# ielhelw/mcmc-ammsb-gpu

Hardware: AMD Instinct MI355X
Metric: mini-batch edges/s (SG-MCMC a-MMSB learner loop) (higher is better)
Workload: dtype f32

## Files before the change

### include/ammsb.h

```cpp
#ifndef AMMSB_H
#define AMMSB_H

#include <stddef.h>
#include <stdint.h>

#ifdef __cplusplus
extern "C" {
#endif

#define AMMSB_VERSION 200

enum {
  AMMSB_OK = 0,
  AMMSB_EINVAL = -1,
  AMMSB_EHIP = -2,
  AMMSB_ENOMEM = -3,
  AMMSB_ENODEV = -4,
  AMMSB_ERANGE = -5
};

#define AMMSB_MAX_GROUPS 65535u
#define AMMSB_RPM_MAX_BLOCKS 32

typedef struct { uint64_t x, y; } ammsb_seed;
// ... 38 lines not shown
int ammsb_ctx_destroy(ammsb_ctx* ctx);
int ammsb_ctx_params(const ammsb_ctx* ctx, ammsb_params* out);

int ammsb_rng_init(ammsb_ctx* ctx, ammsb_seed* seeds, uint64_t n, uint64_t sx, uint64_t sy, void* stream);
int ammsb_rng_init_mixed(ammsb_ctx* ctx, ammsb_seed* seeds, uint64_t n, uint64_t sx, uint64_t sy, void* stream);

int ammsb_set_has(ammsb_ctx* ctx, const ammsb_set* set, const uint64_t* keys, uint64_t n, uint8_t* out,
                  void* stream);

uint64_t ammsb_set_num_bins(uint64_t n);
int ammsb_set_build(ammsb_ctx* ctx, const uint64_t* keys, uint64_t n, uint64_t* slots, uint64_t num_bins,
                    uint32_t* prime_idx_out, uint32_t* scratch, void* stream);

int ammsb_pi_init_gamma(ammsb_ctx* ctx, const ammsb_rpm* pi, float* phi_sum, float eta0, float eta1,
                        ammsb_seed* seeds, void* stream);

int ammsb_sample_neighbors(ammsb_ctx* ctx, ammsb_seed* seeds, const uint32_t* nodes, uint32_t n_nodes,
                           uint32_t wg, uint32_t* table, uint32_t* packed, void* stream);

int ammsb_update_phi(ammsb_ctx* ctx, const float* beta, const ammsb_rpm* pi, const float* phi_sum,
                     const ammsb_set* training_set, const uint32_t* nodes, const uint32_t* neighbors,
                     uint32_t n_nodes, uint32_t step_count, ammsb_seed* seeds, uint32_t wg, uint32_t flags,
                     uint32_t group_begin, uint32_t group_end, float* phi_vec, void* stream);

int ammsb_update_phi_occupancy(ammsb_ctx* ctx, uint32_t wg, int* blocks_per_cu, int* waves_per_block);

int ammsb_update_pi(ammsb_ctx* ctx, const ammsb_rpm* pi, float* phi_sum, const float* phi_vec,
                    const uint32_t* nodes, uint32_t n_nodes, uint32_t wg, void* stream);

int ammsb_theta_sum(ammsb_ctx* ctx, float* out, void* stream);

int ammsb_beta_grads(ammsb_ctx* ctx, const float* theta, const float* beta, const ammsb_rpm* pi,
                     const ammsb_set* training_set, const uint64_t* edges, uint32_t n_edges,
                     uint32_t edge_begin, uint32_t edge_end, uint32_t wg, float* grads_out, void* stream);

int ammsb_can_fuse_pi_beta(ammsb_ctx* ctx, uint32_t phi_wg, uint32_t beta_wg);
int ammsb_update_pi_beta_grads(ammsb_ctx* ctx, const float* theta, const float* beta, const ammsb_rpm* pi,
                               float* phi_sum, const float* phi_vec, const uint32_t* nodes,
                               const ammsb_set* training_set, const uint64_t* edges, uint32_t n_edges, uint32_t wg,
                               float* grads_out, void* stream);

int ammsb_sum_rows_f32(ammsb_ctx* ctx, const float* in, uint32_t rows, uint32_t cols, float* out, void* stream);

int ammsb_update_theta(ammsb_ctx* ctx, float* theta, float* beta, const float* grads, uint32_t step_count,
                       float scale, ammsb_seed* seeds, uint32_t flags, void* stream);

// ... 90 lines not shown
```

### include/mcmc/operators.h

```cpp
#ifndef MCMC_AMD_OPERATORS_H_
#define MCMC_AMD_OPERATORS_H_

#include <functional>
#include <istream>
#include <memory>
#include <ostream>
#include <string>
#include <vector>

#include "ammsb.h"
#include "mcmc/config.h"
#include "mcmc/device.h"

namespace mcmc {

std::shared_ptr<ammsb_ctx> AcquireContext(const Config& cfg, const clcuda::Queue& queue);
void ThrowIfError(ammsb_ctx* ctx, int rc, const char* what);

template <class T>
class RowPartitionedMatrix {
 public:
  RowPartitionedMatrix(clcuda::Queue queue, uint32_t rows, uint32_t cols, uint32_t rows_in_block = 0);
  uint32_t Rows() const { return rows_; }
  uint32_t Cols() const { return cols_; }
// ... 137 lines not shown
    void* stop;
    uint64_t* acc;
  };
  void* Take();
  std::vector<Rec> pending_;
  std::vector<void*> free_;
  void* cur_ = nullptr;
};

class PhiUpdater {
 public:
  PhiUpdater(const Config& cfg, clcuda::Queue queue, clcuda::Buffer<Float>& beta, RowPartitionedMatrix<Float>* pi,
             clcuda::Buffer<Float>& phi, OpenClSet* trainingSet, const std::vector<std::string>& compileFlags = {},
             const std::string& baseFuncs = "");
  void operator()(clcuda::Buffer<Vertex>& mini_batch_nodes, clcuda::Buffer<Vertex>& neighbors,
                  uint32_t num_mini_batch_nodes);
  uint64_t UpdatePhiTime() const { return t_update_phi_; }
  uint64_t UpdatePiTime() const { return t_update_pi_; }
  clcuda::Buffer<Float>& GetPhiVec() { return phi_vec_; }
  void BeginCall() { ++count_calls_; }
  void UpdatePhi(clcuda::Buffer<Vertex>& nodes, clcuda::Buffer<Vertex>& neighbors, uint32_t n, uint32_t group_begin,
                 uint32_t group_end);
  void UpdatePi(clcuda::Buffer<Vertex>& nodes, uint32_t n);
  random::OpenClRandom& Rand() { return rand_; }
  uint32_t& CountCalls() { return count_calls_; }
  uint32_t Local() const { return local_; }
  uint32_t Flags() const { return flags_; }
  void ResolveTimers() { timers_.Resolve(); }
  void AddTimes(uint64_t phi_ns, uint64_t pi_ns) {
    t_update_phi_ += phi_ns;
    t_update_pi_ += pi_ns;
  }
  bool Serialize(std::ostream* out);
  bool Parse(std::istream* in);

 private:
  std::shared_ptr<ammsb_ctx> ctx_;
  clcuda::Queue queue_;
  clcuda::Buffer<Float>& beta_;
  RowPartitionedMatrix<Float>* pi_;
  clcuda::Buffer<Float>& phi_;
  OpenClSet* trainingSet_;
  uint64_t max_nodes_;
  clcuda::Buffer<Float> phi_vec_;
  random::OpenClRandom rand_;
  uint32_t count_calls_, local_, flags_;
// ... 86 lines not shown
```

### mcmc-ammsb-gpu_amd/_capi.py

```python
import ctypes as C
import os

import numpy as np

_HERE = os.path.dirname(os.path.abspath(__file__))
LIB_PATH = os.environ.get("AMMSB_HIP_LIB") or os.path.join(_HERE, "libammsb_hip.so")

RPM_MAX_BLOCKS = 32
MAX_GROUPS = 65535
NOISE_OFF = 1
PHI_STREAMING = 2


class AmmsbError(RuntimeError):
    pass


class Params(C.Structure):
    _fields_ = [("N", C.c_uint64), ("K", C.c_uint64), ("E", C.c_uint64),
                ("num_node_sample", C.c_uint32),
                ("alpha", C.c_float), ("a", C.c_float), ("b", C.c_float), ("c", C.c_float),
                ("epsilon", C.c_float), ("eta0", C.c_float), ("eta1", C.c_float)]


# ... 24 lines not shown
                ("beta_seeds", _vp), ("grads", _vp), ("beta_wg", _u32), ("beta_flags", _u32),
                ("edges", _vp * 2), ("nodes", _vp * 2), ("neighbors", _vp * 2), ("nbr_table", _vp * 2),
                ("nbr_seeds", _vp * 2), ("nbr_wg", _u32),
                ("csr_offsets", _vp), ("csr_targets", _vp), ("mb_seeds", _vp), ("mb_candidates", _u32),
                ("mb_workspace", _vp), ("mb_count", _vp), ("mini_batch", _u32), ("max_fan_out", _u32),
                ("max_nodes", _u32), ("max_edges", _u32), ("flags", _u32)]


class MbChoice(C.Structure):
    _fields_ = [("link", _u32), ("u", _u32), ("n", _u32), ("n_candidates", _u32)]


SIGNATURES = {
    "ammsb_version": [],
    "ammsb_strerror": [C.c_int],
    "ammsb_last_error": [_vp],
    "ammsb_last_kernel_name": [_vp, C.c_int],
    "ammsb_params_quantize": [_P(Params)],
    "ammsb_eps_t": [_P(Params), _u32],
    "ammsb_ctx_create": [C.c_int, _P(Params), _P(_vp)],
    "ammsb_ctx_destroy": [_vp],
    "ammsb_theta_sum": [_vp, _vp, _vp],
    "ammsb_ctx_params": [_vp, _P(Params)],
    "ammsb_rng_init": [_vp, _vp, _u64, _u64, _u64, _vp],
    "ammsb_rng_init_mixed": [_vp, _vp, _u64, _u64, _u64, _vp],
    "ammsb_set_has": [_vp, _P(SetDesc), _vp, _u64, _vp, _vp],
    "ammsb_set_num_bins": [_u64],
    "ammsb_set_build": [_vp, _vp, _u64, _vp, _u64, _P(_u32), _vp, _vp],
    "ammsb_pi_init_gamma": [_vp, _P(Rpm), _vp, _f32, _f32, _vp, _vp],
    "ammsb_sample_neighbors": [_vp, _vp, _vp, _u32, _u32, _vp, _vp, _vp],
    "ammsb_update_phi": [_vp, _vp, _P(Rpm), _vp, _P(SetDesc), _vp, _vp, _u32, _u32, _vp, _u32, _u32,
                         _u32, _u32, _vp, _vp],
    "ammsb_update_phi_occupancy": [_vp, _u32, _P(C.c_int), _P(C.c_int)],
    "ammsb_update_pi": [_vp, _P(Rpm), _vp, _vp, _vp, _u32, _u32, _vp],
    "ammsb_beta_grads": [_vp, _vp, _vp, _P(Rpm), _P(SetDesc), _vp, _u32, _u32, _u32, _u32, _vp, _vp],
    "ammsb_can_fuse_pi_beta": [_vp, _u32, _u32],
    "ammsb_update_pi_beta_grads": [_vp, _vp, _vp, _P(Rpm), _vp, _vp, _vp, _P(SetDesc), _vp, _u32, _u32, _vp, _vp],
    "ammsb_sum_rows_f32": [_vp, _vp, _u32, _u32, _vp, _vp],
    "ammsb_update_theta": [_vp, _vp, _vp, _vp, _u32, _f32, _vp, _u32, _vp],
    "ammsb_beta_from_theta": [_vp, _vp, _vp, _vp],
    "ammsb_perplexity": [_vp, _vp, _P(Rpm), _P(SetDesc), _vp, _u32, _u32, _u32, _u32, _u32, _vp, _vp, _vp],
    "ammsb_minibatch_link": [_vp, _vp, _vp, _u32, _u32, _vp, _vp, _vp],
    "ammsb_minibatch_candidates": [_u64, _u32],
    "ammsb_minibatch_candidates_for": [_u64, _u32, _u64],
    "ammsb_minibatch_workspace_bytes": [_u32],
    "ammsb_minibatch_nonlink": [_vp, _vp, _u32, _u32, _u32, _u32, _P(SetDesc), _P(SetDesc), _vp, _vp, _vp, _vp, _vp],
# ... 96 lines not shown
```

### mcmc-ammsb-gpu_amd/csrc/ammsb_core.hip

```cpp
#include <math.h>
#include <stdlib.h>
#include <string.h>

#include "ammsb_ctx.h"
#include "ammsb_dev.h"
#include "ammsb_step.h"

using namespace ammsb;


extern "C" int ammsb_version(void) { return AMMSB_VERSION; }

extern "C" const char* ammsb_strerror(int code) {
  switch (code) {
    case AMMSB_OK: return "ok";
    case AMMSB_EINVAL: return "invalid argument";
    case AMMSB_EHIP: return "HIP runtime error";
    case AMMSB_ENOMEM: return "out of device memory";
    case AMMSB_ENODEV: return "no usable gfx950 device";
    case AMMSB_ERANGE: return "size out of range for the launch shape";
    default: return "unknown error";
  }
}

// ... 58 lines not shown
  *out = ctx;
  return AMMSB_OK;
}

extern "C" int ammsb_ctx_destroy(ammsb_ctx* ctx) {
  if (!ctx) return AMMSB_EINVAL;
  (void)hipSetDevice(ctx->device);
  if (ctx->grad_partials) (void)hipFree(ctx->grad_partials);
  if (ctx->theta_sum) (void)hipFree(ctx->theta_sum);
  if (ctx->theta_coef) (void)hipFree(ctx->theta_coef);
  if (ctx->ppx_partials) (void)hipFree(ctx->ppx_partials);
  if (ctx->ppx_cnt_partials) (void)hipFree(ctx->ppx_cnt_partials);
  if (ctx->ppx_ticket) (void)hipFree(ctx->ppx_ticket);
  free(ctx);
  return AMMSB_OK;
}

extern "C" int ammsb_ctx_params(const ammsb_ctx* ctx, ammsb_params* out) {
  if (!ctx || !out) return AMMSB_EINVAL;
  *out = ctx->params;
  return AMMSB_OK;
}

static inline uint32_t div_up(uint64_t a, uint64_t b) { return (uint32_t)((a + b - 1) / b); }


__global__ void rng_init_kernel(ammsb_seed* seeds, uint64_t n, uint64_t sx, uint64_t sy) {
  for (uint64_t i = blockIdx.x * (uint64_t)blockDim.x + threadIdx.x; i < n; i += (uint64_t)gridDim.x * blockDim.x) {
    seeds[i].x = sx + i;
    seeds[i].y = sy + i;
  }
}

extern "C" int ammsb_rng_init(ammsb_ctx* ctx, ammsb_seed* seeds, uint64_t n, uint64_t sx, uint64_t sy, void* stream) {
  AMMSB_CHECK_ARG(ctx, ctx && seeds, "null argument");
  if (n == 0) return AMMSB_OK;
  const uint32_t grid = div_up(n, 256) < 4096 ? div_up(n, 256) : 4096;
  rng_init_kernel<<<grid, 256, 0, as_stream(stream)>>>(seeds, n, sx, sy);
  AMMSB_LAUNCH_CHECK(ctx);
  return AMMSB_OK;
}

__device__ __forceinline__ uint64_t splitmix64(uint64_t z) {
  z += 0x9e3779b97f4a7c15ull;
  z = (z ^ (z >> 30)) * 0xbf58476d1ce4e5b9ull;
  z = (z ^ (z >> 27)) * 0x94d049bb133111ebull;
// ... 552 lines not shown
```

### mcmc-ammsb-gpu_amd/csrc/ammsb_ctx.h

```cpp
#pragma once

#include <hip/hip_runtime.h>
#include <stdarg.h>
#include <stdint.h>
#include <stdio.h>

#include <string>

#include "../../include/ammsb.h"

struct ammsb_ctx {
  int device;
  ammsb_params params;
  int num_cus;
  float* grad_partials;
  uint32_t max_partials;
  float* theta_sum;
  float4* theta_coef;
  double* ppx_partials;
  unsigned long long* ppx_cnt_partials;
  uint32_t max_ppx_blocks;
  uint32_t* ppx_ticket;
  const char* kernel_name[7];
  char err[256];
};

enum { AMMSB_KN_PHI = 0, AMMSB_KN_PI = 1, AMMSB_KN_GRADS = 2, AMMSB_KN_PPX = 3, AMMSB_KN_PHI_SMALL = 4, AMMSB_KN_NBR = 5,
       AMMSB_KN_GRADS_SUM = 6 };

static inline std::string ammsb_kname(const char* fmt, ...) {
  char buf[128];
  va_list ap;
  va_start(ap, fmt);
  vsnprintf(buf, sizeof buf, fmt, ap);
  va_end(ap);
  return std::string(buf);
}

#define AMMSB_CHECK_ARG(ctx, cond, msg)                                   \
  do {                                                                    \
    if (!(cond)) {                                                        \
      if (ctx) snprintf((ctx)->err, sizeof((ctx)->err), "%s: %s", __func__, msg); \
      return AMMSB_EINVAL;                                                \
    }                                                                     \
  } while (0)

// ... 30 lines not shown
```

### mcmc-ammsb-gpu_amd/csrc/ammsb_dev.h

```cpp
#pragma once

#include <hip/hip_runtime.h>
#include <stdint.h>

#include "../../include/ammsb.h"

namespace ammsb {


#include "zig_tables.inc"

struct ZigTables {
#ifndef AMMSB_ZIG_YTAB_GLOBAL
  float ytab[128];
#endif
  float wtab[128];
  uint32_t ktab[128];
};

__device__ __forceinline__ void zig_load(ZigTables* t) {
  for (int i = threadIdx.x; i < 128; i += blockDim.x) {
#ifndef AMMSB_ZIG_YTAB_GLOBAL
    t->ytab[i] = zig_ytab[i];
#endif
// ... 185 lines not shown
  FastMod mod;
  uint32_t prime_idx;
};
inline __host__ DevSet dev_set(const ammsb_set& s) {
  return DevSet{s.slots, s.num_bins, fast_mod_init(s.num_bins ? s.num_bins : 1), s.prime_idx};
}

struct SetProbe {
  ulonglong2 a0, a1, c0, c1;
};
__device__ __forceinline__ SetProbe set_probe(const DevSet& set, uint64_t k) {
  const uint64_t h1 = fast_mod(kSetPrimes[2 * set.prime_idx] * k, set.mod);
  const uint64_t h2 = fast_mod(k ^ kSetPrimes[2 * set.prime_idx + 1], set.mod);
  const ulonglong2* b1 = reinterpret_cast<const ulonglong2*>(set.slots + h1 * 4);
  const ulonglong2* b2 = reinterpret_cast<const ulonglong2*>(set.slots + (set.num_bins + h2) * 4);
  return SetProbe{b1[0], b1[1], b2[0], b2[1]};
}
__device__ __forceinline__ bool set_hit(const SetProbe& p, uint64_t k) {
  return (p.a0.x == k) | (p.a0.y == k) | (p.a1.x == k) | (p.a1.y == k) | (p.c0.x == k) | (p.c0.y == k) |
         (p.c1.x == k) | (p.c1.y == k);
}
__device__ __forceinline__ bool set_has(const DevSet& set, uint64_t k) { return set_hit(set_probe(set, k), k); }


__device__ __forceinline__ float* rpm_row(const ammsb_rpm& m, uint64_t row) {
#ifdef AMMSB_RPM_SINGLE
  return reinterpret_cast<float*>(m.blocks[0]) + row * m.num_cols;
#endif
  if (m.num_blocks == 1) return reinterpret_cast<float*>(m.blocks[0]) + row * m.num_cols;
  const uint32_t r = (uint32_t)row, rib = (uint32_t)m.rows_in_block;
  const uint32_t blk = r / rib;
  const uint64_t off = (uint64_t)(r - blk * rib) * m.num_cols;
  return reinterpret_cast<float*>(m.blocks[blk]) + off;
}


template <int L>
struct Group {
  static_assert(L >= 1 && L <= 1024 && (L & (L - 1)) == 0, "L must be a power of two <= 1024");
  static constexpr int BLOCK = L < 64 ? 64 : L;
  static constexpr int PER_BLOCK = BLOCK / L;
  static constexpr int AUX = L > 64 ? 2 * L : 1;

  __device__ __forceinline__ static int lane() { return threadIdx.x & (L - 1); }
  __device__ __forceinline__ static int slot() { return threadIdx.x / L; }

// ... 227 lines not shown
```

### mcmc-ammsb-gpu_amd/csrc/ammsb_phi.hip

```cpp
#pragma clang fp contract(off)

#include <stdlib.h>

#include "ammsb_ctx.h"
#include "ammsb_dev.h"
#include "ammsb_step.h"

#include <type_traits>

using namespace ammsb;

#ifdef AMMSB_PHI_TRACE
__device__ unsigned long long g_phi_trace[256];
#define PHI_TRACE(slot) do { if (blockIdx.x == 0 && threadIdx.x == 0 && (slot) < 256) g_phi_trace[(slot)] = __builtin_readcyclecounter(); } while (0)
extern "C" int ammsb_debug_trace(unsigned long long* out, int n) {
  return hipMemcpyFromSymbol(out, HIP_SYMBOL(g_phi_trace), sizeof(unsigned long long) * (n < 256 ? n : 256)) == hipSuccess ? 0 : -2;
}
#define AMMSB_PHI_BLK_CAP 65536
__device__ unsigned long long g_phi_blk[AMMSB_PHI_BLK_CAP * 5];
#define PHI_BLK(end) do { if (threadIdx.x == 0 && blockIdx.x < AMMSB_PHI_BLK_CAP) { \
    g_phi_blk[blockIdx.x * 5 + (end)] = __builtin_readcyclecounter(); \
    g_phi_blk[blockIdx.x * 5 + 2 + (end)] = __builtin_amdgcn_s_memrealtime(); \
    if (!(end)) g_phi_blk[blockIdx.x * 5 + 4] = (unsigned long long)__builtin_amdgcn_s_getreg((31 << 11) | 4) | \
                                               ((unsigned long long)__builtin_amdgcn_s_getreg((31 << 11) | 20) << 32); } } while (0)
// ... 7 lines not shown

#ifndef AMMSB_PHI_LDS3_DEFAULT
#define AMMSB_PHI_LDS3_DEFAULT false
#endif

namespace {

struct PhiArgs {
  const float* beta;
  ammsb_rpm pi;
  const float* phi_sum;
  DevSet set;
  const uint32_t* nodes;
  const uint32_t* neighbors;
  ammsb_seed* seeds;
  float* phi_vec;
  uint32_t n_nodes, G, group_begin, group_end;
  uint32_t K, n;
  float eps_t, alpha, epsilon, Nn;
  uint32_t noise_on;
  uint32_t rows_nt;
  const ammsb_step_desc* desc;
  unsigned long long* stamps;
};


struct PhiStep {
  uint32_t n_nodes, G, group_end;
  float eps_t;
};
__device__ __forceinline__ PhiStep phi_step(const PhiArgs& a) {
  PhiStep st = {a.n_nodes, a.G, a.group_end, a.eps_t};
  if (a.desc) {
    st.n_nodes = a.desc->n_nodes;
    st.G = st.n_nodes < AMMSB_MAX_GROUPS ? st.n_nodes : AMMSB_MAX_GROUPS;
    st.group_end = st.G;
    st.eps_t = a.desc->eps_t;
  }
  return st;
}

template <int L, int KPT, int DEPTH, bool FULL, bool ONE = false>
__global__ __launch_bounds__(Group<L>::BLOCK) void update_phi_kernel(const PhiArgs a) {
  if constexpr (ONE) __builtin_assume(a.pi.num_blocks == 1);
  using Grp = Group<L>;
  extern __shared__ uint32_t s_nb_all[];
  __shared__ ZigTables zig;
// ... 361 lines not shown
  auto group_sum = [&](float v) -> float {
    if constexpr (W == 1) {
      return VLn::tree(v);
    } else {
      float* x = xsum + phase * L;
      phase ^= 1;
      x[tid] = v;
      __syncthreads();
      float part[W];
#pragma unroll
      for (int i = 0; i < W; ++i) part[i] = x[64 * i + ln];
#pragma unroll
      for (int st = W / 2; st >= 1; st >>= 1) {
#pragma unroll
        for (int i = 0; i < st; ++i) part[i] += part[i + st];
      }
      return Group<64>::wave_tree64(part[0]);
    }
  };

  for (uint64_t i = g; i < st.n_nodes; i += st.G) {
    const uint32_t node = a.nodes[i];
    group_sync();
    for (uint32_t q = tid; q < n; q += L) {
      const uint32_t nbq = a.neighbors[i * n + q];
      const bool y = set_has(a.set, make_edge(node, nbq));
      s_nb[q] = nbq | (y ? 0x80000000u : 0u);
    }
    group_sync();

    const float phi_sum = a.phi_sum[node];
    const float inv_phi_sum = 1.0f / phi_sum;
    const float* row_a = rpm_row(a.pi, node);
    f32x2 pi_a[HP], grads[HP], rden[HP];
    bool node_safe = beta_safe && in_range(phi_sum, kPhiSumLo, kPhiSumHi);
#pragma unroll
    for (int p = 0; p < HP; ++p)
      pi_a[p] = f32x2{__builtin_nontemporal_load(row_a + tid + 2 * L * p), __builtin_nontemporal_load(row_a + tid + 2 * L * p + L)};
#pragma unroll
    for (uint32_t r = 0; r < (uint32_t)(D - 1); ++r)
      if (r < n) request(r, r);
#pragma unroll
    for (int p = 0; p < HP; ++p) {
      grads[p] = f32x2{0.0f, 0.0f};
      const f32x2 den = pi_a[p] * phi_sum;
      rden[p] = f32x2{exact_rcp(den.x), exact_rcp(den.y)};
      node_safe = node_safe && in_range(den.x, kDenLo, kDenHi) && in_range(den.y, kDenLo, kDenHi);
      const f32x2 ep = den * st.eps_t;
      s_noise[ln + 128 * p] = sqrtf(ep.x);
      s_noise[ln + 128 * p + 64] = sqrtf(ep.y);
// ... 62 lines not shown
          f32x2 qv = div_exact3(pr, psum2, rps2);
          qv = div_exact3(qv, pi_a[p] * ps, rden[p]);
          grads[p] += qv - inv_phi_sum;
        }
      } else {
#pragma unroll
        for (int p = 0; p < HP; ++p) {
          const f32x2 den = pi_a[p] * phi_sum;
          float q0 = row[ln + 128 * p] / probs_sum;
          float q1 = row[ln + 128 * p + 64] / probs_sum;
          q0 = q0 / den.x;
          q1 = q1 / den.y;
          grads[p] += f32x2{q0 - inv_phi_sum, q1 - inv_phi_sum};
        }
      }
    }

    if (a.noise_on) {
#pragma unroll 1
      for (uint32_t j = D > 2 ? n : (n > 0 ? n - 1 : 0); j < (uint32_t)KV; ++j) draw_normal(j);
    }
    asm volatile("s_waitcnt lgkmcnt(0)" ::: "memory");

    float* out = a.phi_vec + i * K;
    const float half = st.eps_t / 2;
#pragma unroll
    for (int p = 0; p < HP; ++p) {
      const f32x2 bb = f32x2{s_noise[ln + 128 * p], s_noise[ln + 128 * p + 64]};
      const f32x2 phi_k = pi_a[p] * phi_sum;
      const f32x2 ng = grads[p] * a.Nn;
      f32x2 in = a.alpha - phi_k;
      in = in + ng;
      const f32x2 drift = in * half;
      const f32x2 aa = phi_k + drift;
      const f32x2 s2 = aa + bb;
      const float v0 = fabsf(s2.x), v1 = fabsf(s2.y);
      __builtin_nontemporal_store(v0 > 1e-24f ? v0 : 1e-24f, out + tid + 2 * L * p);
      __builtin_nontemporal_store(v1 > 1e-24f ? v1 : 1e-24f, out + tid + 2 * L * p + L);
    }
  }
  if (a.noise_on && tid < LV) a.seeds[(uint64_t)g * LV + tid] = rs;
  PHI_BLK(1);
}

template <int KPT, int VL = 64, bool ONE = false>
__global__ __launch_bounds__(64) __attribute__((amdgpu_waves_per_eu(3))) void update_phi_lds3_kernel(const PhiArgs a) {
  if constexpr (ONE) __builtin_assume(a.pi.num_blocks == 1);
  using VLn = VLane<VL>;
  constexpr int D = 3;
  constexpr int KV = KPT * VLn::PER;
  constexpr int L = 64, KW = 64 * KPT, K = L * KPT, PIECES = KPT / 4, HP = KPT / 2;
  extern __shared__ __align__(16) char smem[];
  __shared__ ZigTables zig;
  const int tid = threadIdx.x, ln = tid;
  const uint32_t n = a.n;
  float* ring = reinterpret_cast<float*>(smem);
  uint32_t* s_nb = reinterpret_cast<uint32_t*>(smem + D * KW * sizeof(float));

  const PhiStep st = phi_step(a);
  note_stamp(a.stamps, a.desc, AMMSB_STAMP_PHI);
  const uint32_t g = a.group_begin + blockIdx.x;
// ... 202 lines not shown

  auto request = [&](uint32_t q, uint32_t slot) {
    const uint32_t nbr = __builtin_amdgcn_readfirstlane(s_nb[q] & 0x7fffffffu);
    const float* src = rpm_row(a.pi, nbr) + 4 * tid;
    char* dst = smem + slot * (KW * sizeof(float));
    if (a.rows_nt) {
#pragma unroll
      for (int t = 0; t < PIECES; ++t)
        __builtin_amdgcn_global_load_lds((glb_void_t*)(src + 4 * L * t), (lds_void_t*)(dst + 1024 * t), 16, 0, 2);
    } else {
#pragma unroll
      for (int t = 0; t < PIECES; ++t)
        __builtin_amdgcn_global_load_lds((glb_void_t*)(src + 4 * L * t), (lds_void_t*)(dst + 1024 * t), 16, 0, 0);
    }
  };

  PHI_TRACE(0);
  for (uint32_t g = g0; g < st.group_end; g += gridDim.x) {
  if (a.noise_on) rs = a.seeds[(uint64_t)g * VL + VLn::vlane(tid)];
  for (uint64_t i = g; i < st.n_nodes; i += st.G) {
    const uint32_t node = a.nodes[i];
    __syncthreads();
    for (uint32_t q = tid; q < n; q += L) s_nb[q] = a.neighbors[i * n + q];
    __syncthreads();
    PHI_TRACE(1);

    const float phi_sum = a.phi_sum[node];
    const float inv_phi_sum = 1.0f / phi_sum;
    const float* row_a = rpm_row(a.pi, node);
    f32x2 pi_a[HP], grads[HP], rden[HP];
    bool node_safe = beta_safe && in_range(phi_sum, kPhiSumLo, kPhiSumHi);
#pragma unroll
    for (int p = 0; p < HP; ++p)
      pi_a[p] = f32x2{__builtin_nontemporal_load(row_a + tid + 2 * L * p), __builtin_nontemporal_load(row_a + tid + 2 * L * p + L)};
#pragma unroll
    for (uint32_t r = 0; r < (uint32_t)(D - U); ++r)
      if (r < n) request(r, r);
    const bool one_probe = n <= (uint32_t)L;
    const uint32_t my_nb = one_probe && (uint32_t)tid < n ? s_nb[tid] : 0u;
    SetProbe my_probe = {};
    if (one_probe && (uint32_t)tid < n) my_probe = set_probe(a.set, make_edge(node, my_nb));
    float zraw[REGN ? KV : 1];
    if constexpr (REGN) {
      if (a.noise_on) {
#pragma unroll
        for (int j = 0; j < KV; ++j) zraw[j] = rng_normal(rs, &zig);
      }
    }
    if (one_probe) {
      if ((uint32_t)tid < n && set_hit(my_probe, make_edge(node, my_nb))) s_nb[tid] = my_nb | 0x80000000u;
    } else {
      for (uint32_t q = tid; q < n; q += L) {
        const uint32_t nb = s_nb[q];
        if (set_has(a.set, make_edge(node, nb))) s_nb[q] = nb | 0x80000000u;
      }
    }
    __syncthreads();
    PHI_TRACE(2);
#pragma unroll
    for (int p = 0; p < HP; ++p) {
      grads[p] = f32x2{0.0f, 0.0f};
      const f32x2 den = pi_a[p] * phi_sum;
      rden[p] = f32x2{exact_rcp(den.x), exact_rcp(den.y)};
      node_safe = node_safe && in_range(den.x, kDenLo, kDenHi) && in_range(den.y, kDenLo, kDenHi);
      const f32x2 ep = den * st.eps_t;
      if constexpr (REGN) {
        nz[2 * p] = sqrtf(ep.x);
        nz[2 * p + 1] = sqrtf(ep.y);
      } else {
        s_noise[ln + 128 * p] = sqrtf(ep.x);
        s_noise[ln + 128 * p + 64] = sqrtf(ep.y);
      }
    }

    PHI_TRACE(3);
    for (uint32_t q = 0; q < n; q += U) {
      float* row[U];
// ... 433 lines not shown

  const PhiStep st = phi_step(a);
  note_stamp(a.stamps, a.desc, AMMSB_STAMP_PHI);
  const uint32_t g = a.group_begin + blockIdx.x;
  if (g >= st.group_end) return;
  const float EPS = a.epsilon;
  if (a.noise_on) zig_load(&zig);

  float bf[KPT];
  bool beta_safe = true;
#pragma unroll
  for (int j = 0; j < KPT; ++j) {
    const float b = a.beta[2 * (ln + 64 * j) + 1];
    bf[j] = b - EPS;
    beta_safe = beta_safe && in_range(b, EPS, kBetaHi);
  }
  ammsb_seed rs = {0, 0};
  const bool noise_wave = wv == RW;
  if (a.noise_on && noise_wave) rs = a.seeds[(uint64_t)g * VL + VLn::vlane(ln)];

  for (uint64_t i = g; i < st.n_nodes; i += st.G) {
    const uint32_t node = a.nodes[i];
    __syncthreads();
    for (uint32_t q = tid; q < n; q += T) {
      const uint32_t nbq = a.neighbors[i * n + q];
      const bool y = set_has(a.set, make_edge(node, nbq));
      s_nb[q] = nbq | (y ? 0x80000000u : 0u);
    }
    const float phi_sum = a.phi_sum[node];
    const float inv_phi_sum = 1.0f / phi_sum;
    const float* row_a = rpm_row(a.pi, node);
    float pi_a[KPT], rden[KPT];
    bool node_safe = beta_safe && in_range(phi_sum, kPhiSumLo, kPhiSumHi);
#pragma unroll
    for (int j = 0; j < KPT; ++j) pi_a[j] = row_a[ln + 64 * j];
    if (noise_wave) {
#pragma unroll
      for (int j = 0; j < KPT; ++j) s_pia[ln + 64 * j] = pi_a[j];
    } else {
#pragma unroll
      for (int j = 0; j < KPT; ++j) {
        const float den = pi_a[j] * phi_sum;
        rden[j] = exact_rcp(den);
        node_safe = node_safe && in_range(den, kDenLo, kDenHi);
      }
    }
    __syncthreads();

    if (!noise_wave) {
      float cur[KPT], nxt[KPT];
// ... 890 lines not shown
  if (generic && gen_threads(p.K, wg, 1) == 0) {
    snprintf(ctx->err, sizeof ctx->err, "ammsb_update_phi: K=%llu at wg=%u: more than 32 columns per work-item needs K <= %u",
             (unsigned long long)p.K, wg, kGenMaxK);
    return AMMSB_ERANGE;
  }
  PhiArgs a;
  a.beta = beta;
  a.pi = *pi;
  a.phi_sum = phi_sum;
  a.set = dev_set(*training_set);
  a.nodes = nodes;
  a.neighbors = neighbors;
  a.seeds = seeds;
  a.phi_vec = phi_vec;
  a.n_nodes = n_nodes;
  a.G = n_nodes < AMMSB_MAX_GROUPS ? n_nodes : AMMSB_MAX_GROUPS;
  a.group_begin = group_begin;
  a.group_end = group_end < a.G ? group_end : a.G;
  a.K = (uint32_t)p.K;
  a.n = p.num_node_sample;
  a.eps_t = desc ? 0.0f : ammsb_eps_t(&p, step_count);
  a.desc = desc;
  a.stamps = stamps;
  a.alpha = p.alpha;
  a.epsilon = p.epsilon;
  a.Nn = (1.0f * (float)p.N) / (float)p.num_node_sample;
  a.noise_on = (flags & AMMSB_NOISE_OFF) ? 0u : 1u;
  {
    static const int nt_mode = [] {
      const char* f = getenv("AMMSB_PHI_NT");
      return f ? atoi(f) : -1;
    }();
    const uint64_t pi_bytes = pi->num_rows * pi->num_cols * sizeof(float);
    a.rows_nt = nt_mode >= 0 ? (uint32_t)nt_mode : (pi_bytes > (256ull << 20) ? 1u : 0u);
  }
  if (a.group_begin >= a.group_end) return AMMSB_OK;
  const uint32_t n_groups = a.group_end - a.group_begin;
  hipStream_t s = as_stream(stream);
  static const bool lds3_env = [] {
    const char* f = getenv("AMMSB_PHI_LDS3");
    return f ? atoi(f) != 0 : AMMSB_PHI_LDS3_DEFAULT;
  }();
  const bool lds3 = g_phi_form_lds3 >= 0 ? g_phi_form_lds3 != 0 : lds3_env;
  static const bool force_reg = [] {
    const char* f = getenv("AMMSB_PHI_FORM");
    return f && f[0] == 'r';
// ... 199 lines not shown
```

### mcmc-ammsb-gpu_amd/host/learner.cc

```cpp
#include "mcmc/learner.h"
#include "mcmc/exchange.h"
#include "mcmc/serialize.h"
#include "ammsb_refsample.h"

#include <hip/hip_runtime.h>

#include <algorithm>
#include <chrono>
#include <cmath>
#include <cstring>
#include <functional>
#include <iostream>
#include <random>
#include <sstream>
#include <stdexcept>
#include <string>
#include <tuple>

using namespace std::chrono;

namespace mcmc {

namespace {
clcuda::Buffer<Edge> Upload(const clcuda::Queue& q, const std::vector<Edge>& v) {
// ... 58 lines not shown
    trainingPerplexity_.reset(new PerplexityCalculator(PerplexityCalculator::EDGE_PER_WORKGROUP, cfg_, queue_, beta_,
                                                       pi_.get(), *devTrainingPerplexityEdges_, trainingSet_.get()));
  }
  samples_[0].reset(new Sample(cfg_, queue_, cfg_.sample_seed[0]));
  samples_[1].reset(new Sample(cfg_, queue_, cfg_.sample_seed[1]));
  if (cfg_.sampling_stream != "own" && cfg_.sampling_stream != "reference")
    throw std::runtime_error("sampling_stream must be own or reference (got " + cfg_.sampling_stream + ")");
  ref_stream_ = cfg_.device_sampling && cfg_.sampling_stream == "reference";
  if (ref_stream_ && cfg_.graph_launch)
    throw std::runtime_error("graph_launch does not cover sampling_stream reference: the descriptor loop needs each "
                             "mini-batch's sizes before the device has drawn it");
  if (cfg_.device_sampling) {
    if (cfg_.strategy != Node && cfg_.strategy != NodeLink && cfg_.strategy != NodeNonLink)
      throw std::runtime_error("device sampling implements Node / NodeLink / NodeNonLink only");
    ctx_ = AcquireContext(cfg_, queue_);
    std::vector<uint64_t> off;
    std::vector<Vertex> tgt;
    cfg_.trainingGraph->ExportCSR(&off, &tgt);
    if (tgt.empty()) throw std::runtime_error("training graph has no edges");
    degree_.resize(cfg_.N);
    for (uint64_t u = 0; u < cfg_.N; ++u) degree_[u] = static_cast<uint32_t>(off[u + 1] - off[u]);
    csr_offsets_.reset(new clcuda::Buffer<uint64_t>(queue_.GetContext(), queue_, off.begin(), off.end()));
    csr_targets_.reset(new clcuda::Buffer<Vertex>(queue_.GetContext(), queue_, tgt.begin(), tgt.end()));
    excluded_.assign(cfg_.N, 1);
    uint32_t max_excluded = 1;
    for (uint64_t u = 0; u < cfg_.N; ++u) excluded_[u] += degree_[u];
    if (cfg_.heldout)
      for (Edge e : cfg_.heldout_edges)
        if (cfg_.heldout->Has(e)) {
          Vertex a, b;
          std::tie(a, b) = Vertices(e);
          ++excluded_[a];
          ++excluded_[b];
        }
    for (uint64_t u = 0; u < cfg_.N; ++u) max_excluded = std::max(max_excluded, excluded_[u]);
    candidates_ = CandidatesForExcluded(max_excluded);
    if (candidates_ == 0)
      throw std::runtime_error("device sampling needs N >= 2 * mini_batch with room for the largest degree");
    if (ref_stream_) {
      for (uint64_t u = 0; u < cfg_.N; ++u)
        for (uint64_t i = off[u]; i < off[u + 1]; ++i)
          if (tgt[i] == u) throw std::runtime_error("reference-stream sampling: the training graph holds a self-loop");
      const uint64_t items = std::max<uint64_t>(cfg_.mini_batch_size, cfg_.trainingGraph->MaxFanOut()) + 1;
      ammsb_refsample* h = nullptr;
      const int rc = ammsb_refsample_create(queue_.device(), cfg_.N, static_cast<uint32_t>(cfg_.mini_batch_size),
                                            candidates_, static_cast<uint32_t>(items), &h);
// ... 836 lines not shown
```

### mcmc-ammsb-gpu_amd/host/operators.cc

```cpp
#include "mcmc/operators.h"
#include "mcmc/exchange.h"
#include "mcmc/serialize.h"

#include <hip/hip_runtime.h>

#include <algorithm>
#include <iostream>
#include <cstring>
#include <map>
#include <mutex>
#include <stdexcept>
#include <tuple>

namespace mcmc {

void ThrowIfError(ammsb_ctx* ctx, int rc, const char* what) {
  if (rc == AMMSB_OK) return;
  throw std::runtime_error(std::string(what) + ": " + ammsb_strerror(rc) + " (" + ammsb_last_error(ctx) + ")");
}

std::shared_ptr<ammsb_ctx> AcquireContext(const Config& cfg, const clcuda::Queue& queue) {
  const ammsb_params p = MakeKernelParams(cfg);
  ammsb_ctx* ctx = nullptr;
  const int rc = ammsb_ctx_create(queue.device(), &p, &ctx);
// ... 268 lines not shown
  return cfg;
}

PhiUpdater::PhiUpdater(const Config& cfg, clcuda::Queue queue, clcuda::Buffer<Float>& beta,
                       RowPartitionedMatrix<Float>* pi, clcuda::Buffer<Float>& phi, OpenClSet* trainingSet,
                       const std::vector<std::string>&, const std::string&)
    : ctx_(AcquireContext(CheckedPhiConfig(cfg), queue)),
      queue_(queue),
      beta_(beta),
      pi_(pi),
      phi_(phi),
      trainingSet_(trainingSet),
      max_nodes_(MaxNodes(cfg)),
      phi_vec_(queue.GetContext(), PhiVecRows(cfg) * cfg.K),
      rand_(queue, max_nodes_ * cfg.phi_wg_size, cfg.phi_seed),
      count_calls_(0),
      local_(cfg.phi_wg_size),
      flags_(cfg.phi_disable_noise ? AMMSB_NOISE_OFF : 0u),
      async_(cfg.async_launch),
      timed_(cfg.async_launch && cfg.loop_timers && !cfg.graph_launch),
      t_update_phi_(0),
      t_update_pi_(0) {}

void PhiUpdater::operator()(clcuda::Buffer<Vertex>& nodes, clcuda::Buffer<Vertex>& neighbors, uint32_t n) {
  if (n == 0) throw std::runtime_error("mini-batch nodes size = 0!");
  if (n > max_nodes_) throw std::runtime_error("grads too small");
  ++count_calls_;
  if (async_) {
    if (timed_) timers_.Start(queue_.stream());
    ThrowIfError(ctx_.get(),
                 ammsb_update_phi(ctx_.get(), beta_.data(), &pi_->Get(), phi_.data(), &trainingSet_->Get(), nodes.data(),
                                  neighbors.data(), n, count_calls_, rand_.Get(), local_, flags_, 0, 0xFFFFFFFFu,
                                  phi_vec_.data(), queue_.stream()),
                 "ammsb_update_phi");
    if (timed_) {
      timers_.Stop(queue_.stream(), &t_update_phi_);
      timers_.Start(queue_.stream());
    }
    ThrowIfError(ctx_.get(),
                 ammsb_update_pi(ctx_.get(), &pi_->Get(), phi_.data(), phi_vec_.data(), nodes.data(), n, local_,
                                 queue_.stream()),
                 "ammsb_update_pi");
    if (timed_) timers_.Stop(queue_.stream(), &t_update_pi_);
    return;
  }
  {
// ... 238 lines not shown
```

### mcmc-ammsb-gpu_amd/learner.py

```python
import concurrent.futures
import os
import time

import numpy as np
import torch

from ._capi import AmmsbError, MAX_GROUPS
from .postfit import PostFit


class Config:

    def __init__(self, **kw):
        self.heldout_ratio = 0.01
        self.alpha = 0.001
        self.a, self.b, self.c = 0.0315, 1024.0, 0.5
        self.epsilon = 1e-7
        self.eta0, self.eta1 = 1.0, 1.0
        self.K = 32
        self.mini_batch_size = 32
        self.num_node_sample = 32
        self.N = 0
        self.E = 0
        self.ppx_wg_size = 32
# ... 160 lines not shown
        if cfg.sample_parallel:
            self.samples.append(Sample(self, cfg.sample_seeds[1]))
        self.phase = 0
        self.futures = [None, None]
        self.pool = (concurrent.futures.ThreadPoolExecutor(max_workers=1)
                     if not cfg.device_sampling or self.ref_stream else None)
        self.dev_sampler = None
        self.ref_sampler = None
        self.loop = None
        self._loop_dirty = False
        if cfg.device_sampling:
            off, tgt = dataset.training_csr()
            he = np.ascontiguousarray(dataset.heldout_edges, dtype=np.uint64)
            he = he[dataset.heldout.Has(he)] if he.size else he
            ends = np.concatenate([he >> np.uint64(32), he & np.uint64(0xFFFFFFFF)]).astype(np.int64)
            hdeg = np.bincount(ends, minlength=N)[:N]
            if self.ref_stream:
                self.ref_sampler = ops.ReferenceStreamSampler(c, off, tgt, self.trainingSet, self.heldoutSet,
                                                              cfg.mini_batch_size, heldout_degree=hdeg)
            else:
                self.dev_sampler = ops.DeviceMiniBatchSampler(c, off, tgt, self.trainingSet, self.heldoutSet,
                                                              cfg.mini_batch_size, cfg.device_sampling_seed,
                                                              heldout_degree=hdeg)
        self.grads_mode, self.grads_fused = "sharded", False
        if self.sharded:
            want = str(getattr(cfg, "beta_grads", "auto"))
            if want not in ("auto", "sharded", "replicated"):
                raise AmmsbError("beta_grads must be auto, sharded or replicated (got %r)" % (want,))
            fusable = (self.dev_sampler is not None and cfg.strategy in ("Node", "NodeLink", "NodeNonLink")
                       and hasattr(self.betaUpdater, "can_fuse_update_pi")
                       and self.betaUpdater.can_fuse_update_pi(self.phiUpdater))
            self.grads_mode = "replicated" if want == "replicated" or (want == "auto" and fusable) else "sharded"
            self.grads_fused = fusable
        if self.sharded:
            self.rep_stream = ops.new_stream(c)
            self.ev_fork, self.ev_join = ops.new_event(), ops.new_event()
            self.all_grads = c.zeros((self.world, 2 * K), torch.float32)
            self.grads_sum = c.zeros((2 * K,), torch.float32)
            self.all_sums = c.zeros((self.world, 4), torch.int64)
            self.tail_buf = c.zeros((max(max_nodes - MAX_GROUPS, 1), K), torch.float32)
        from . import hostlib
        self.theta.copy_(c.from_numpy(hostlib.theta_init(K, cfg.eta0, cfg.eta1)))
        ops.beta_from_theta(c, self.theta, self.beta)
        ops.RandomGammaAndNormalize(c, cfg.eta0, cfg.eta1, self.pi, self.phi)
        self.pi_placement = None
        self._place_pi()
# ... 661 lines not shown
```

### mcmc-ammsb-gpu_amd/ops.py

```python
import ctypes as C
import os
import threading

import numpy as np
import torch

from . import _capi
from ._capi import AmmsbError, NOISE_OFF, PHI_STREAMING, Params, PpxSums, Rpm, SetDesc, check

SEED_DT = np.dtype([("x", np.uint64), ("y", np.uint64)])


_tls = threading.local()


def _stream():
    stack = getattr(_tls, "stack", None)
    if stack:
        return stack[-1]
    return C.c_void_p(torch.cuda.current_stream().cuda_stream)


def _torch_stream():
    stack = getattr(_tls, "tstack", None)
# ... 58 lines not shown
        if not torch.cuda.is_available():
            raise AmmsbError("no HIP device visible: the MI355X path has no CPU fallback")
        self.lib = _capi.load()
        self.device = torch.device("cuda", torch.cuda.current_device() if device is None else device)
        self.params = params
        self._ctx = C.c_void_p()
        check(self.lib.ammsb_ctx_create(self.device.index, C.byref(params), C.byref(self._ctx)))

    @property
    def handle(self):
        return self._ctx

    def check(self, rc):
        check(rc, self._ctx)

    KERNELS = ("update_phi", "update_pi", "beta_grads", "perplexity", "update_phi_small", "sample_neighbors",
               "grads_sum")

    def kernel_names(self):
        names = {k: self.lib.ammsb_last_kernel_name(self.handle, i).decode() for i, k in enumerate(self.KERNELS)}
        if not names["update_phi"]:
            names["update_phi"] = names["update_phi_small"]
        return names

    def close(self):
        if self._ctx:
            self.lib.ammsb_ctx_destroy(self._ctx)
            self._ctx = C.c_void_p()

    def __del__(self):
        try:
            self.close()
        except Exception:
            pass

    def empty(self, shape, dtype):
        return torch.empty(shape, dtype=dtype, device=self.device)

    def zeros(self, shape, dtype):
        return torch.zeros(shape, dtype=dtype, device=self.device)

    def from_numpy(self, arr):
        a = np.ascontiguousarray(arr)
        if a.dtype == np.uint64:
            a = a.view(np.int64)
        elif a.dtype == np.uint32:
# ... 1165 lines not shown
```

Baseline: 36.33 million.

## Test phi neighbor link flags against CSR adjacency rows instead of hash set

Registers the training graph CSR (offsets/targets) with the context and, in the update_phi kernels, decides whether each sampled neighbor is a training link by scanning the node's adjacency row with wavefront readlane broadcasts and XOR-min comparisons, for rows of degree up to 256. Nodes with larger degree, and configurations with the AMMSB_PHI_FLAGS=s env override, keep the hash-set probe. The aim is to replace scattered hash-table probes with a coalesced read of one contiguous row. It adds a scan cost proportional to degree, plus kernarg reloads of the set and adjacency pointers through the kernarg segment. A small output-pointer tweak in the store loop keeps tid in a vector register.

```diff
diff --git a/include/ammsb.h b/include/ammsb.h
--- a/include/ammsb.h
+++ b/include/ammsb.h
@@ -84,6 +84,8 @@
                      const ammsb_set* training_set, const uint32_t* nodes, const uint32_t* neighbors,
                      uint32_t n_nodes, uint32_t step_count, ammsb_seed* seeds, uint32_t wg, uint32_t flags,
                      uint32_t group_begin, uint32_t group_end, float* phi_vec, void* stream);
+
+int ammsb_ctx_set_training_adjacency(ammsb_ctx* ctx, const uint64_t* offsets, const uint32_t* targets);
 
 int ammsb_update_phi_occupancy(ammsb_ctx* ctx, uint32_t wg, int* blocks_per_cu, int* waves_per_block);
 
diff --git a/include/mcmc/operators.h b/include/mcmc/operators.h
--- a/include/mcmc/operators.h
+++ b/include/mcmc/operators.h
@@ -183,6 +183,7 @@
   void UpdatePhi(clcuda::Buffer<Vertex>& nodes, clcuda::Buffer<Vertex>& neighbors, uint32_t n, uint32_t group_begin,
                  uint32_t group_end);
   void UpdatePi(clcuda::Buffer<Vertex>& nodes, uint32_t n);
+  void SetTrainingAdjacency(const uint64_t* offsets, const Vertex* targets);
   random::OpenClRandom& Rand() { return rand_; }
   uint32_t& CountCalls() { return count_calls_; }
   uint32_t Local() const { return local_; }
diff --git a/mcmc-ammsb-gpu_amd/_capi.py b/mcmc-ammsb-gpu_amd/_capi.py
--- a/mcmc-ammsb-gpu_amd/_capi.py
+++ b/mcmc-ammsb-gpu_amd/_capi.py
@@ -70,6 +70,7 @@
     "ammsb_ctx_destroy": [_vp],
     "ammsb_theta_sum": [_vp, _vp, _vp],
     "ammsb_ctx_params": [_vp, _P(Params)],
+    "ammsb_ctx_set_training_adjacency": [_vp, _vp, _vp],
     "ammsb_rng_init": [_vp, _vp, _u64, _u64, _u64, _vp],
     "ammsb_rng_init_mixed": [_vp, _vp, _u64, _u64, _u64, _vp],
     "ammsb_set_has": [_vp, _P(SetDesc), _vp, _u64, _vp, _vp],
diff --git a/mcmc-ammsb-gpu_amd/csrc/ammsb_core.hip b/mcmc-ammsb-gpu_amd/csrc/ammsb_core.hip
--- a/mcmc-ammsb-gpu_amd/csrc/ammsb_core.hip
+++ b/mcmc-ammsb-gpu_amd/csrc/ammsb_core.hip
@@ -104,6 +104,14 @@
   return AMMSB_OK;
 }
 
+extern "C" int ammsb_ctx_set_training_adjacency(ammsb_ctx* ctx, const uint64_t* offsets, const uint32_t* targets) {
+  AMMSB_CHECK_ARG(ctx, ctx, "null context");
+  AMMSB_CHECK_ARG(ctx, (offsets == nullptr) == (targets == nullptr), "offsets and targets: both or neither");
+  ctx->adj_offsets = offsets;
+  ctx->adj_targets = targets;
+  return AMMSB_OK;
+}
+
 static inline uint32_t div_up(uint64_t a, uint64_t b) { return (uint32_t)((a + b - 1) / b); }
 
 
diff --git a/mcmc-ammsb-gpu_amd/csrc/ammsb_ctx.h b/mcmc-ammsb-gpu_amd/csrc/ammsb_ctx.h
--- a/mcmc-ammsb-gpu_amd/csrc/ammsb_ctx.h
+++ b/mcmc-ammsb-gpu_amd/csrc/ammsb_ctx.h
@@ -22,6 +22,8 @@
   uint32_t max_ppx_blocks;
   uint32_t* ppx_ticket;
   const char* kernel_name[7];
+  const uint64_t* adj_offsets;
+  const uint32_t* adj_targets;
   char err[256];
 };
 
diff --git a/mcmc-ammsb-gpu_amd/csrc/ammsb_dev.h b/mcmc-ammsb-gpu_amd/csrc/ammsb_dev.h
--- a/mcmc-ammsb-gpu_amd/csrc/ammsb_dev.h
+++ b/mcmc-ammsb-gpu_amd/csrc/ammsb_dev.h
@@ -231,6 +231,46 @@
 }
 __device__ __forceinline__ bool set_has(const DevSet& set, uint64_t k) { return set_hit(set_probe(set, k), k); }
 
+constexpr uint32_t kAdjRowCap = 256;
+
+struct AdjRow {
+  const uint32_t* row;
+  uint32_t deg;
+  __device__ __forceinline__ bool usable() const { return deg <= kAdjRowCap; }
+};
+__device__ __forceinline__ AdjRow adj_row(const uint64_t* offsets, const uint32_t* targets, uint32_t node) {
+  AdjRow r = {nullptr, kAdjRowCap + 1};
+  if (offsets) {
+    typedef unsigned long long u64x2 __attribute__((ext_vector_type(2), aligned(8)));
+    const u64x2 o = *reinterpret_cast<const u64x2*>(offsets + node);
+    const uint64_t d = o.y - o.x;
+    const uint64_t p = reinterpret_cast<uint64_t>(targets + o.x);
+    const uint32_t lo = __builtin_amdgcn_readfirstlane((uint32_t)p), hi = __builtin_amdgcn_readfirstlane((uint32_t)(p >> 32));
+    r.row = reinterpret_cast<const uint32_t*>(((uint64_t)hi << 32) | lo);
+    r.deg = __builtin_amdgcn_readfirstlane(d <= kAdjRowCap ? (uint32_t)d : kAdjRowCap + 1);
+  }
+  return r;
+}
+__device__ __forceinline__ uint32_t adj_chunk(const AdjRow& r, uint32_t c0, uint32_t lane) {
+  const uint32_t k = c0 + lane;
+  return r.row[k < r.deg ? k : r.deg - 1];
+}
+__device__ __forceinline__ uint32_t adj_scan(uint32_t t, uint32_t m, uint32_t id, uint32_t miss) {
+  for (uint32_t j = 0; j < m; ++j) {
+    const uint32_t x = (uint32_t)__builtin_amdgcn_readlane((int)t, (int)j) ^ id;
+    miss = x < miss ? x : miss;
+  }
+  return miss;
+}
+__device__ __forceinline__ bool adj_has(const AdjRow& r, uint32_t lane, uint32_t id, uint32_t t0) {
+  uint32_t miss = adj_scan(t0, r.deg < 64 ? r.deg : 64, id, 0xFFFFFFFFu);
+  for (uint32_t c0 = 64; c0 < r.deg; c0 += 64) miss = adj_scan(adj_chunk(r, c0, lane), r.deg - c0 < 64 ? r.deg - c0 : 64, id, miss);
+  return miss == 0;
+}
+__device__ __forceinline__ bool adj_has(const AdjRow& r, uint32_t lane, uint32_t id) {
+  return r.deg ? adj_has(r, lane, id, adj_chunk(r, 0, lane)) : false;
+}
+
 
 __device__ __forceinline__ float* rpm_row(const ammsb_rpm& m, uint64_t row) {
 #ifdef AMMSB_RPM_SINGLE
diff --git a/mcmc-ammsb-gpu_amd/csrc/ammsb_phi.hip b/mcmc-ammsb-gpu_amd/csrc/ammsb_phi.hip
--- a/mcmc-ammsb-gpu_amd/csrc/ammsb_phi.hip
+++ b/mcmc-ammsb-gpu_amd/csrc/ammsb_phi.hip
@@ -53,7 +53,33 @@
   uint32_t rows_nt;
   const ammsb_step_desc* desc;
   unsigned long long* stamps;
+  const uint64_t* adj_offsets;
+  const uint32_t* adj_targets;
 };
+
+struct PhiFlagArgs {
+  DevSet set;
+  const uint64_t* adj_offsets;
+  const uint32_t* adj_targets;
+};
+typedef const __attribute__((address_space(4))) char* kernarg_ptr_t;
+__device__ __forceinline__ uint64_t kernarg_u64(kernarg_ptr_t ka, size_t off) {
+  return *reinterpret_cast<const __attribute__((address_space(4))) uint64_t*>(ka + off);
+}
+__device__ __forceinline__ PhiFlagArgs phi_flag_args() {
+  kernarg_ptr_t ka = (kernarg_ptr_t)__builtin_amdgcn_kernarg_segment_ptr();
+  asm volatile("" : "+s"(ka));
+  constexpr size_t S = offsetof(PhiArgs, set);
+  PhiFlagArgs f;
+  f.set.slots = reinterpret_cast<const uint64_t*>(kernarg_u64(ka, S + offsetof(DevSet, slots)));
+  f.set.num_bins = kernarg_u64(ka, S + offsetof(DevSet, num_bins));
+  f.set.mod.d = kernarg_u64(ka, S + offsetof(DevSet, mod) + offsetof(FastMod, d));
+  f.set.mod.m = kernarg_u64(ka, S + offsetof(DevSet, mod) + offsetof(FastMod, m));
+  f.set.prime_idx = (uint32_t)kernarg_u64(ka, S + offsetof(DevSet, prime_idx));
+  f.adj_offsets = reinterpret_cast<const uint64_t*>(kernarg_u64(ka, offsetof(PhiArgs, adj_offsets)));
+  f.adj_targets = reinterpret_cast<const uint32_t*>(kernarg_u64(ka, offsetof(PhiArgs, adj_targets)));
+  return f;
+}
 
 
 struct PhiStep {
@@ -461,10 +487,29 @@
   for (uint64_t i = g; i < st.n_nodes; i += st.G) {
     const uint32_t node = a.nodes[i];
     group_sync();
-    for (uint32_t q = tid; q < n; q += L) {
-      const uint32_t nbq = a.neighbors[i * n + q];
-      const bool y = set_has(a.set, make_edge(node, nbq));
-      s_nb[q] = nbq | (y ? 0x80000000u : 0u);
+    if constexpr (KPT <= 16 && W <= 4) {
+      const PhiFlagArgs fa = phi_flag_args();
+      const AdjRow adj = adj_row(fa.adj_offsets, fa.adj_targets, node);
+      if (adj.usable()) {
+        for (uint32_t q0 = 64 * wv; q0 < n; q0 += L) {
+          const uint32_t q = q0 + ln;
+          const uint32_t nbq = a.neighbors[i * n + (q < n ? q : n - 1)];
+          const bool y = adj_has(adj, (uint32_t)ln, nbq);
+          if (q < n) s_nb[q] = nbq | (y ? 0x80000000u : 0u);
+        }
+      } else {
+        for (uint32_t q = tid; q < n; q += L) {
+          const uint32_t nbq = a.neighbors[i * n + q];
+          const bool y = set_has(fa.set, make_edge(node, nbq));
+          s_nb[q] = nbq | (y ? 0x80000000u : 0u);
+        }
+      }
+    } else {
+      for (uint32_t q = tid; q < n; q += L) {
+        const uint32_t nbq = a.neighbors[i * n + q];
+        const bool y = set_has(a.set, make_edge(node, nbq));
+        s_nb[q] = nbq | (y ? 0x80000000u : 0u);
+      }
     }
     group_sync();
 
@@ -573,7 +618,9 @@
     }
     asm volatile("s_waitcnt lgkmcnt(0)" ::: "memory");
 
-    float* out = a.phi_vec + i * K;
+    uint32_t tid_out = (uint32_t)tid;
+    if constexpr (KPT <= 16) asm volatile("" : "+v"(tid_out));
+    float* out = a.phi_vec + i * K + tid_out;
     const float half = st.eps_t / 2;
 #pragma unroll
     for (int p = 0; p < HP; ++p) {
@@ -586,8 +633,8 @@
       const f32x2 aa = phi_k + drift;
       const f32x2 s2 = aa + bb;
       const float v0 = fabsf(s2.x), v1 = fabsf(s2.y);
-      __builtin_nontemporal_store(v0 > 1e-24f ? v0 : 1e-24f, out + tid + 2 * L * p);
-      __builtin_nontemporal_store(v1 > 1e-24f ? v1 : 1e-24f, out + tid + 2 * L * p + L);
+      __builtin_nontemporal_store(v0 > 1e-24f ? v0 : 1e-24f, out + 2 * L * p);
+      __builtin_nontemporal_store(v1 > 1e-24f ? v1 : 1e-24f, out + 2 * L * p + L);
     }
   }
   if (a.noise_on && tid < LV) a.seeds[(uint64_t)g * LV + tid] = rs;
@@ -836,6 +883,8 @@
     const uint32_t node = a.nodes[i];
     __syncthreads();
     for (uint32_t q = tid; q < n; q += L) s_nb[q] = a.neighbors[i * n + q];
+    const PhiFlagArgs fa = phi_flag_args();
+    const AdjRow adj = adj_row(fa.adj_offsets, fa.adj_targets, node);
     __syncthreads();
     PHI_TRACE(1);
 
@@ -850,10 +899,13 @@
 #pragma unroll
     for (uint32_t r = 0; r < (uint32_t)(D - U); ++r)
       if (r < n) request(r, r);
-    const bool one_probe = n <= (uint32_t)L;
+    const bool by_row = adj.usable();
+    const bool one_probe = !by_row && n <= (uint32_t)L;
     const uint32_t my_nb = one_probe && (uint32_t)tid < n ? s_nb[tid] : 0u;
     SetProbe my_probe = {};
-    if (one_probe && (uint32_t)tid < n) my_probe = set_probe(a.set, make_edge(node, my_nb));
+    if (one_probe && (uint32_t)tid < n) my_probe = set_probe(fa.set, make_edge(node, my_nb));
+    uint32_t my_target = 0;
+    if (by_row && adj.deg) my_target = adj_chunk(adj, 0, (uint32_t)tid);
     float zraw[REGN ? KV : 1];
     if constexpr (REGN) {
       if (a.noise_on) {
@@ -861,12 +913,21 @@
         for (int j = 0; j < KV; ++j) zraw[j] = rng_normal(rs, &zig);
       }
     }
-    if (one_probe) {
+    if (by_row) {
+      if (adj.deg) {
+        for (uint32_t q0 = 0; q0 < n; q0 += L) {
+          const uint32_t q = q0 + tid;
+          const uint32_t nbq = s_nb[q < n ? q : n - 1];
+          const bool y = adj_has(adj, (uint32_t)tid, nbq, my_target);
+          if (q < n && y) s_nb[q] = nbq | 0x80000000u;
+        }
+      }
+    } else if (one_probe) {
       if ((uint32_t)tid < n && set_hit(my_probe, make_edge(node, my_nb))) s_nb[tid] = my_nb | 0x80000000u;
     } else {
       for (uint32_t q = tid; q < n; q += L) {
         const uint32_t nb = s_nb[q];
-        if (set_has(a.set, make_edge(node, nb))) s_nb[q] = nb | 0x80000000u;
+        if (set_has(fa.set, make_edge(node, nb))) s_nb[q] = nb | 0x80000000u;
       }
     }
     __syncthreads();
@@ -1346,10 +1407,21 @@
   for (uint64_t i = g; i < st.n_nodes; i += st.G) {
     const uint32_t node = a.nodes[i];
     __syncthreads();
-    for (uint32_t q = tid; q < n; q += T) {
-      const uint32_t nbq = a.neighbors[i * n + q];
-      const bool y = set_has(a.set, make_edge(node, nbq));
-      s_nb[q] = nbq | (y ? 0x80000000u : 0u);
+    const PhiFlagArgs fa = phi_flag_args();
+    const AdjRow adj = adj_row(fa.adj_offsets, fa.adj_targets, node);
+    if (adj.usable()) {
+      for (uint32_t q0 = 64 * wv; q0 < n; q0 += T) {
+        const uint32_t q = q0 + ln;
+        const uint32_t nbq = a.neighbors[i * n + (q < n ? q : n - 1)];
+        const bool y = adj_has(adj, (uint32_t)ln, nbq);
+        if (q < n) s_nb[q] = nbq | (y ? 0x80000000u : 0u);
+      }
+    } else {
+      for (uint32_t q = tid; q < n; q += T) {
+        const uint32_t nbq = a.neighbors[i * n + q];
+        const bool y = set_has(fa.set, make_edge(node, nbq));
+        s_nb[q] = nbq | (y ? 0x80000000u : 0u);
+      }
     }
     const float phi_sum = a.phi_sum[node];
     const float inv_phi_sum = 1.0f / phi_sum;
@@ -2286,6 +2358,15 @@
   a.eps_t = desc ? 0.0f : ammsb_eps_t(&p, step_count);
   a.desc = desc;
   a.stamps = stamps;
+  {
+    static const bool flags_from_set = [] {
+      const char* f = getenv("AMMSB_PHI_FLAGS");
+      return f && f[0] == 's';
+    }();
+    const bool rows = ctx->adj_offsets && !flags_from_set;
+    a.adj_offsets = rows ? ctx->adj_offsets : nullptr;
+    a.adj_targets = rows ? ctx->adj_targets : nullptr;
+  }
   a.alpha = p.alpha;
   a.epsilon = p.epsilon;
   a.Nn = (1.0f * (float)p.N) / (float)p.num_node_sample;
diff --git a/mcmc-ammsb-gpu_amd/host/learner.cc b/mcmc-ammsb-gpu_amd/host/learner.cc
--- a/mcmc-ammsb-gpu_amd/host/learner.cc
+++ b/mcmc-ammsb-gpu_amd/host/learner.cc
@@ -104,6 +104,9 @@
     for (uint64_t u = 0; u < cfg_.N; ++u) degree_[u] = static_cast<uint32_t>(off[u + 1] - off[u]);
     csr_offsets_.reset(new clcuda::Buffer<uint64_t>(queue_.GetContext(), queue_, off.begin(), off.end()));
     csr_targets_.reset(new clcuda::Buffer<Vertex>(queue_.GetContext(), queue_, tgt.begin(), tgt.end()));
+    phiUpdater_.SetTrainingAdjacency(csr_offsets_->data(), csr_targets_->data());
+    ThrowIfError(ctx_.get(), ammsb_ctx_set_training_adjacency(ctx_.get(), csr_offsets_->data(), csr_targets_->data()),
+                 "ammsb_ctx_set_training_adjacency");
     excluded_.assign(cfg_.N, 1);
     uint32_t max_excluded = 1;
     for (uint64_t u = 0; u < cfg_.N; ++u) excluded_[u] += degree_[u];
diff --git a/mcmc-ammsb-gpu_amd/host/operators.cc b/mcmc-ammsb-gpu_amd/host/operators.cc
--- a/mcmc-ammsb-gpu_amd/host/operators.cc
+++ b/mcmc-ammsb-gpu_amd/host/operators.cc
@@ -314,6 +314,11 @@
       t_update_phi_(0),
       t_update_pi_(0) {}
 
+void PhiUpdater::SetTrainingAdjacency(const uint64_t* offsets, const Vertex* targets) {
+  ThrowIfError(ctx_.get(), ammsb_ctx_set_training_adjacency(ctx_.get(), offsets, targets),
+               "ammsb_ctx_set_training_adjacency");
+}
+
 void PhiUpdater::operator()(clcuda::Buffer<Vertex>& nodes, clcuda::Buffer<Vertex>& neighbors, uint32_t n) {
   if (n == 0) throw std::runtime_error("mini-batch nodes size = 0!");
   if (n > max_nodes_) throw std::runtime_error("grads too small");
diff --git a/mcmc-ammsb-gpu_amd/learner.py b/mcmc-ammsb-gpu_amd/learner.py
--- a/mcmc-ammsb-gpu_amd/learner.py
+++ b/mcmc-ammsb-gpu_amd/learner.py
@@ -206,6 +206,8 @@
                 self.dev_sampler = ops.DeviceMiniBatchSampler(c, off, tgt, self.trainingSet, self.heldoutSet,
                                                               cfg.mini_batch_size, cfg.device_sampling_seed,
                                                               heldout_degree=hdeg)
+            sampler = self.ref_sampler or self.dev_sampler
+            c.set_training_adjacency(sampler.offsets, sampler.targets)
         self.grads_mode, self.grads_fused = "sharded", False
         if self.sharded:
             want = str(getattr(cfg, "beta_grads", "auto"))
diff --git a/mcmc-ammsb-gpu_amd/ops.py b/mcmc-ammsb-gpu_amd/ops.py
--- a/mcmc-ammsb-gpu_amd/ops.py
+++ b/mcmc-ammsb-gpu_amd/ops.py
@@ -104,6 +104,10 @@
         if not names["update_phi"]:
             names["update_phi"] = names["update_phi_small"]
         return names
+
+    def set_training_adjacency(self, offsets, targets):
+        self.check(self.lib.ammsb_ctx_set_training_adjacency(self.handle, _ptr(offsets), _ptr(targets)))
+        self._adjacency = (offsets, targets)
 
     def close(self):
         if self._ctx:
```

After: 36.07 million. About the same (-0.7%).
